# mgaido91/FBK-fairseq-ST

Hardware: AMD Instinct MI355X
Metric: audio-frames/sec (train fwd+bwd) s2t_transformer_m, 80-mel (higher is better)
Workload: dtype bf16

## Files before the change

### fbk_fairseq_st_amd/csrc/attention.hip

```cpp
#include "common.hpp"
#include "prof.hpp"
#include <cstdlib>
#include <type_traits>

template <typename T, int DH> struct ACfg {
    static constexpr int E = Elem<T>::PER16;
    static constexpr int ROWB = DH * (int)sizeof(T);
    static constexpr int NCH = ROWB / 16;
    static constexpr int KG = NCH / 4;
    static constexpr int PROWB = 64 * (int)sizeof(T);
    static constexpr int PCH = PROWB / 16;
    static constexpr int PKG = PCH / 4;
    static constexpr int ND = DH / 16;
    static constexpr int TILE = 64 * ROWB;
    static constexpr int TTILE = DH * PROWB;
    static constexpr int PTILE = 16 * PROWB;
};

__device__ __forceinline__ int swz(int row, int c, int nch) { return c ^ (row & ((nch < 8 ? nch : 8) - 1)); }

template <typename T, int DH>
__device__ __forceinline__ void stage_rows(char* lds, const T* g, long stride, int row0, int nvalid) {
    typedef ACfg<T, DH> C;
    for (int cid = threadIdx.x; cid < 64 * C::NCH; cid += 256) {
// ... 703 lines not shown
        for (int n = 0; n < 4; ++n) { dkT[kb][n] = (f32x4){0.f, 0.f, 0.f, 0.f}; dvT[kb][n] = dkT[kb][n]; }
    const uint32_t drop_th16 = (uint32_t)fminf(p.p_drop * 4294967296.f, 4294967295.f) >> 16;
    const float drop_inv = 1.f / (1.f - p.p_drop);
    const uint32_t drop_ks = drop_seed_key(p.seed), drop_hwm = drop_high_mix(p.seed, 0);
    const uint32_t tkq = (uint32_t)((p.Tk + 3) >> 2);
    const uint32_t drop_thm1x2 = (drop_th16 - 1u) * 0x00010001u;
    const uint32_t own_bit = ((r16 & 1) ? 0x00010000u : 1u) << ((r16 >> 1) & 1);

    const int qstart = p.causal ? bx * 128 : 0;
    const int ntile = qstart < p.Tq ? (p.Tq - qstart + 63) / 64 : 0;
    float* sStat = reinterpret_cast<float*>(smem + 32768);
    auto stage = [&](int qt, int stg) {
        stage2_dma(Qg, p.q_st, dOg, p.do_st, qt, p.Tq, smem + stg * 16384, wave, lane);
        if (wave < 2) {
            float* dst = sStat + stg * 128 + wave * 64;
            if (wave == 1 || qt + lane < p.Tq) {
                const char* sb = reinterpret_cast<const char*>(wave == 0 ? lse : dlt);
                const char* src = sb + (uint32_t)(min(qt + lane, p.Tq - 1) * 4);
                __builtin_amdgcn_global_load_lds((__attribute__((address_space(1))) const void*)src,
                                                 (__attribute__((address_space(3))) void*)dst, 4, 0, 0);
            } else dst[lane] = INFINITY;
        }
    };
    if (ntile > 0) stage(qstart, 0);
    {
        u32x4 kk[4], vv[4];
#pragma unroll
        for (int i = 0; i < 4; ++i) {
            const int cid = threadIdx.x + 256 * i, row = cid >> 3, c = cid & 7;
            const long key = min(bx * 128 + row, p.Tk - 1);
            kk[i] = *reinterpret_cast<const u32x4*>(Kg + key * p.k_st + c * 8);
            vv[i] = *reinterpret_cast<const u32x4*>(Vg + key * p.v_st + c * 8);
        }
#pragma unroll
        for (int i = 0; i < 4; ++i) {
            const int cid = threadIdx.x + 256 * i, row = cid >> 3, c = cid & 7;
            const bool in = bx * 128 + row < klen;
#pragma unroll
            for (int w = 0; w < 4; ++w) { kk[i][w] = in ? kk[i][w] : 0u; vv[i][w] = in ? vv[i][w] : 0u; }
            *reinterpret_cast<u32x4*>(sKown + row * 128 + ((c ^ (row & 7)) << 4)) = kk[i];
            *reinterpret_cast<u32x4*>(sVown + row * 128 + ((c ^ (row & 7)) << 4)) = vv[i];
        }
    }
    S2T_WAIT_VM0();
    __syncthreads();
    const float sc2 = p.scale * 1.44269504088896f;
    const bool generic = p.causal || p.dist_pen;
    ASTAMP(7, 1)
    for (int t = 0; t < ntile; ++t) {
        const int qt = qstart + t * 64;
        const char* sQ = smem + (t & 1) * 16384;
        const char* sDO = sQ + 8192;
        const float* sL = sStat + (t & 1) * 128;
        ASTAMP(t, 0)
        if (t + 1 < ntile) stage(qt + 64, (t + 1) & 1);
        ASTAMP(t, 1)
        auto tile = [&](auto edge_tag, auto drop_tag) {
        constexpr bool EDGE = decltype(edge_tag)::value, DROP = decltype(drop_tag)::value;
#pragma unroll 1
        for (int ib = 0; ib < 2; ++ib) {
        u32x4 pf[2], sf[2];
#pragma unroll
        for (int ii = 0; ii < 2; ++ii) {
            const int i = 2 * ib + ii;
            u32x4 qa[2], da[2];
#pragma unroll
            for (int g = 0; g < 2; ++g) { qa[g] = row_frag128(sQ, 16 * i + r16, 4 * g + q); da[g] = row_frag128(sDO, 16 * i + r16, 4 * g + q); }
            const f32x4 L = *reinterpret_cast<const f32x4*>(sL + 16 * i + 4 * q) * 1.44269504088896f;
            const f32x4 Dl = *reinterpret_cast<const f32x4*>(sL + 64 + 16 * i + 4 * q);
            const uint32_t qrow_quads = DROP ? (uint32_t)(((b * p.H + h) * p.Tq + qt + 16 * i + 4 * q + (r16 & 3))) * tkq : 0u;
#pragma unroll
            for (int kb = 0; kb < 2; ++kb) {
                f32x4 st = {0.f, 0.f, 0.f, 0.f}, dp = {0.f, 0.f, 0.f, 0.f};
#pragma unroll
                for (int g = 0; g < 2; ++g) {
                    const int krow = wave * 32 + 16 * kb + r16;
                    st = mma16<bf16>(qa[g], row_frag128(sKown, krow, 4 * g + q), st);
                    dp = mma16<bf16>(da[g], row_frag128(sVown, krow, 4 * g + q), dp);
                }
                const int key = kw + 16 * kb + r16;
                uint32_t nib = 0u;
                if constexpr (DROP) {
                    const u32x2 hq = drop_hash4_lo(drop_ks, drop_hwm, qrow_quads + ((uint32_t)key >> 2));
                    uint32_t dy, dx, ky, kx;
                    asm("v_pk_sub_u16 %0, %1, %2 clamp" : "=v"(dy) : "v"(hq[1]), "v"(drop_thm1x2));
                    asm("v_pk_sub_u16 %0, %1, %2 clamp" : "=v"(dx) : "v"(hq[0]), "v"(drop_thm1x2));
                    asm("v_pk_min_u16 %0, %1, %2" : "=v"(ky) : "v"(dy), "v"(0x00010001u));
                    asm("v_pk_min_u16 %0, %1, %2" : "=v"(kx) : "v"(dx), "v"(0x00010001u));
                    nib = drop_th16 > 0 ? (ky | (kx << 1)) : 0x00030003u;
                }
                float pv[4], ds[4];
#pragma unroll
                for (int r = 0; r < 4; ++r) {
                    const int qrow = qt + 16 * i + 4 * q + r;
                    float arg = __builtin_fmaf(st[r], sc2, -L[r]);
                    if constexpr (EDGE) { if (p.dist_pen) arg -= dist_pen_log2(qrow, key); }
                    float e = __builtin_amdgcn_exp2f(arg);
                    if constexpr (EDGE) e = (qrow < p.Tq && (!p.causal || key <= qrow)) ? e : 0.f;
                    if constexpr (DROP) {
                        const bool keep = (quad_bcast(nib, r) & own_bit) != 0u;
                        pv[r] = keep ? e : 0.f;
                        ds[r] = e * __builtin_fmaf(keep ? dp[r] : 0.f, drop_inv, -Dl[r]);
                    } else {
                        pv[r] = e;
                        ds[r] = e * (dp[r] - Dl[r]);
                    }
                }
                pf[kb][2 * ii] = pack_bf16(pv[0], pv[1]); pf[kb][2 * ii + 1] = pack_bf16(pv[2], pv[3]);
                sf[kb][2 * ii] = pack_bf16(ds[0], ds[1]); sf[kb][2 * ii + 1] = pack_bf16(ds[2], ds[3]);
            }
        }
#pragma unroll
            for (int n = 0; n < 4; ++n) {
                const u32x4 dot = tr_frag128(sDO, ib, n, r16, q), qtf = tr_frag128(sQ, ib, n, r16, q);
#pragma unroll
                for (int kb = 0; kb < 2; ++kb) {
                    dvT[kb][n] = mma16<bf16>(dot, pf[kb], dvT[kb][n]);
                    dkT[kb][n] = mma16<bf16>(qtf, sf[kb], dkT[kb][n]);
                }
            }
        }
        };
        const bool edge = generic;
        if (p.p_drop > 0.f) { if (edge) tile(std::true_type{}, std::true_type{}); else tile(std::false_type{}, std::true_type{}); }
        else if (edge) tile(std::true_type{}, std::false_type{});
        else tile(std::false_type{}, std::false_type{});
        ASTAMP(t, 3)
        S2T_WAIT_VM0();
        ASTAMP(t, 4)
        __syncthreads();
        ASTAMP(t, 5)
    }
    ASTAMP(7, 2)
    const float dv_scale = p.p_drop > 0.f ? drop_inv : 1.f;
    bf16* dKg = reinterpret_cast<bf16*>(p.dK) + (long)b * p.dk_sb + (long)h * DH;
    bf16* dVg = reinterpret_cast<bf16*>(p.dV) + (long)b * p.dv_sb + (long)h * DH;
#pragma unroll
    for (int kb = 0; kb < 2; ++kb) {
        const int key = kw + 16 * kb + r16;
        if (key >= p.Tk) continue;
        const float kz = key < klen ? 1.f : 0.f;
#pragma unroll
        for (int n = 0; n < 4; ++n) { dkT[kb][n] *= kz * p.scale; dvT[kb][n] *= kz * dv_scale; }
#pragma unroll
        for (int n = 0; n < 4; ++n) {
            u32x2 w;
            w[0] = pack_bf16(dkT[kb][n][0], dkT[kb][n][1]); w[1] = pack_bf16(dkT[kb][n][2], dkT[kb][n][3]);
            *reinterpret_cast<u32x2*>(dKg + (long)key * p.dk_st + 16 * n + 4 * q) = w;
            w[0] = pack_bf16(dvT[kb][n][0], dvT[kb][n][1]); w[1] = pack_bf16(dvT[kb][n][2], dvT[kb][n][3]);
            *reinterpret_cast<u32x2*>(dVg + (long)key * p.dv_st + 16 * n + 4 * q) = w;
        }
    }
    ASTAMP(7, 3)
}

__global__ __launch_bounds__(256, 2) void attn_bwd_dq2_kernel(AttnArgs p) {
    constexpr int DH = 64;
    ASTAMP_EARLY(1)
    extern __shared__ __attribute__((aligned(16))) char smem[];
    const int lane = threadIdx.x & 63, wave = threadIdx.x >> 6, r16 = lane & 15, q = lane >> 4;
    int head;
    const int bx = head_xcd_remap(head, p.B * p.H, gridDim.x);
    const int b = head / p.H, h = head % p.H, qw = bx * 128 + wave * 32;
    const int klen = p.klen ? min(p.klen[b], p.Tk) : p.Tk;
    const bf16* Qg = reinterpret_cast<const bf16*>(p.Q) + (long)b * p.q_sb + (long)h * DH;
    const bf16* Kg = reinterpret_cast<const bf16*>(p.K) + (long)b * p.k_sb + (long)h * DH;
    const bf16* Vg = reinterpret_cast<const bf16*>(p.V) + (long)b * p.v_sb + (long)h * DH;
    const bf16* dOg = reinterpret_cast<const bf16*>(p.dO) + (long)b * p.do_sb + (long)h * DH;
    const float* lse = p.LSE + ((long)b * p.H + h) * p.Tq;
    const float* dlt = p.Delta + ((long)b * p.H + h) * p.Tq;

    int kv_end = klen;
    if (p.causal) kv_end = min(kv_end, bx * 128 + 128);
    const int ntile = (kv_end + 63) / 64;
    if (ntile > 0) stage2_dma(Kg, p.k_st, Vg, p.v_st, 0, p.Tk, smem, wave, lane);
    u32x4 qf[2][2], dof[2][2];
    float L[2], Dl[2];
    const bf16* Og = reinterpret_cast<const bf16*>(p.O) + (long)b * p.o_sb + (long)h * DH;
    u32x4 of[2][2];
#pragma unroll
    for (int qb = 0; qb < 2; ++qb) {
        const long row = min(qw + 16 * qb + r16, p.Tq - 1);
        L[qb] = lse[row] * 1.44269504088896f;
#pragma unroll
        for (int g = 0; g < 2; ++g) {
            qf[qb][g] = *reinterpret_cast<const u32x4*>(Qg + row * p.q_st + (4 * g + q) * 8);
            dof[qb][g] = *reinterpret_cast<const u32x4*>(dOg + row * p.do_st + (4 * g + q) * 8);
            of[qb][g] = *reinterpret_cast<const u32x4*>(Og + row * p.o_st + (4 * g + q) * 8);
        }
    }
#pragma unroll
    for (int qb = 0; qb < 2; ++qb) {
        const int row = qw + 16 * qb + r16;
        const bool in = row < p.Tq;
        float part = 0.f;
#pragma unroll
        for (int g = 0; g < 2; ++g) {
#pragma unroll
            for (int w = 0; w < 4; ++w) { qf[qb][g][w] = in ? qf[qb][g][w] : 0u; dof[qb][g][w] = in ? dof[qb][g][w] : 0u; }
            const bf16* oe = reinterpret_cast<const bf16*>(&of[qb][g]);
            const bf16* de = reinterpret_cast<const bf16*>(&dof[qb][g]);
#pragma unroll
            for (int e = 0; e < 8; ++e) part += (float)oe[e] * (float)de[e];
        }
        L[qb] = in ? L[qb] : 0.f;
        part += __shfl_xor(part, 16); part += __shfl_xor(part, 32);
        Dl[qb] = part;
        if (q == 0 && in) const_cast<float*>(dlt)[row] = part;
    }
    f32x4 dqT[2][4];
#pragma unroll
    for (int qb = 0; qb < 2; ++qb)
#pragma unroll
        for (int n = 0; n < 4; ++n) dqT[qb][n] = (f32x4){0.f, 0.f, 0.f, 0.f};
    const uint32_t drop_th16 = (uint32_t)fminf(p.p_drop * 4294967296.f, 4294967295.f) >> 16;
    const float drop_inv = 1.f / (1.f - p.p_drop);
    const uint32_t drop_ks = drop_seed_key(p.seed), drop_hwm = drop_high_mix(p.seed, 0);
    const uint32_t tkq = (uint32_t)((p.Tk + 3) >> 2);

    const float sc2 = p.scale * 1.44269504088896f;
    const bool generic = p.causal || p.dist_pen;
    S2T_WAIT_VM0();
    __syncthreads();
    ASTAMP(7, 1)
    for (int t = 0; t < ntile; ++t) {
        const int kv0 = t * 64;
        const char* sK = smem + (t & 1) * 16384;
        const char* sV = sK + 8192;
        ASTAMP(t, 0)
        if (t + 1 < ntile) stage2_dma(Kg, p.k_st, Vg, p.v_st, kv0 + 64, p.Tk, smem + ((t + 1) & 1) * 16384, wave, lane);
        ASTAMP(t, 1)
        u32x4 sf[2][2];
        auto ds_tile = [&](auto edge_tag, auto drop_tag, auto tail_tag) {
        constexpr bool EDGE = decltype(edge_tag)::value, DROP = decltype(drop_tag)::value, TAIL = decltype(tail_tag)::value;
        const int tail_thr = klen - kv0 - 4 * q;
#pragma unroll
        for (int j = 0; j < 4; ++j) {
            u32x4 ka[2], va[2];
#pragma unroll
            for (int g = 0; g < 2; ++g) { ka[g] = row_frag128(sK, 16 * j + r16, 4 * g + q); va[g] = row_frag128(sV, 16 * j + r16, 4 * g + q); }
#pragma unroll
            for (int qb = 0; qb < 2; ++qb) {
                f32x4 st = {0.f, 0.f, 0.f, 0.f}, dp = {0.f, 0.f, 0.f, 0.f};
#pragma unroll
                for (int g = 0; g < 2; ++g) { st = mma16<bf16>(ka[g], qf[qb][g], st); dp = mma16<bf16>(va[g], dof[qb][g], dp); }
                const int qrow = qw + 16 * qb + r16;
                const int key0 = kv0 + 16 * j + 4 * q;
                u32x2 hq = {0u, 0u};
                if constexpr (DROP) hq = drop_hash4_lo(drop_ks, drop_hwm, (uint32_t)((b * p.H + h) * p.Tq + qrow) * tkq + ((uint32_t)key0 >> 2));
                float ds[4];
#pragma unroll
                for (int r = 0; r < 4; ++r) {
                    float arg = __builtin_fmaf(st[r], sc2, -L[qb]);
                    if constexpr (EDGE) { if (p.dist_pen) arg -= dist_pen_log2(qrow, key0 + r); }
                    float e = __builtin_amdgcn_exp2f(arg);
                    if constexpr (EDGE) {
                        const int key = key0 + r;
                        e = (key < klen && (!p.causal || key <= qrow)) ? e : 0.f;
                    }
                    if constexpr (TAIL) e = (16 * j + r < tail_thr) ? e : 0.f;
                    if constexpr (DROP) ds[r] = e * __builtin_fmaf(drop_field(hq, r) >= drop_th16 ? dp[r] : 0.f, drop_inv, -Dl[qb]);
                    else ds[r] = e * (dp[r] - Dl[qb]);
                }
                sf[qb][j >> 1][2 * (j & 1)] = pack_bf16(ds[0], ds[1]); sf[qb][j >> 1][2 * (j & 1) + 1] = pack_bf16(ds[2], ds[3]);
            }
        }
        };
        const bool tail = kv0 + 64 > klen;
        if (generic) { if (p.p_drop > 0.f) ds_tile(std::true_type{}, std::true_type{}, std::false_type{}); else ds_tile(std::true_type{}, std::false_type{}, std::false_type{}); }
        else if (p.p_drop > 0.f) { if (tail) ds_tile(std::false_type{}, std::true_type{}, std::true_type{}); else ds_tile(std::false_type{}, std::true_type{}, std::false_type{}); }
        else if (tail) ds_tile(std::false_type{}, std::false_type{}, std::true_type{});
        else ds_tile(std::false_type{}, std::false_type{}, std::false_type{});
        ASTAMP(t, 2)
#pragma unroll
        for (int jb = 0; jb < 2; ++jb)
#pragma unroll
            for (int n = 0; n < 4; ++n) {
                const u32x4 kt = tr_frag128(sK, jb, n, r16, q);
#pragma unroll
                for (int qb = 0; qb < 2; ++qb) dqT[qb][n] = mma16<bf16>(kt, sf[qb][jb], dqT[qb][n]);
            }
        ASTAMP(t, 3)
        S2T_WAIT_VM0();
        ASTAMP(t, 4)
        __syncthreads();
        ASTAMP(t, 5)
    }
    ASTAMP(7, 2)
    bf16* dQg = reinterpret_cast<bf16*>(p.dQ) + (long)b * p.dq_sb + (long)h * DH;
#pragma unroll
    for (int qb = 0; qb < 2; ++qb) {
        const int qrow = qw + 16 * qb + r16;
        if (qrow >= p.Tq) continue;
#pragma unroll
        for (int n = 0; n < 4; ++n) {
            u32x2 w;
            w[0] = pack_bf16(dqT[qb][n][0] * p.scale, dqT[qb][n][1] * p.scale); w[1] = pack_bf16(dqT[qb][n][2] * p.scale, dqT[qb][n][3] * p.scale);
            *reinterpret_cast<u32x2*>(dQg + (long)qrow * p.dq_st + 16 * n + 4 * q) = w;
        }
    }
    ASTAMP(7, 3)
}

static bool span32(long stride, int rows) {
    return stride >= 0 && stride * 2 < (1l << 24) && (long)rows * stride * 2 + 256 < (1l << 32);
}
static bool strides_ok(int dtype, const long* s, int n) {
    const int e = dtype == S2T_BF16 ? 8 : 4;
    for (int i = 0; i < n; ++i) if (s[i] % e) return false;
    return true;
}

template <typename T, int DH> static int fwd_launch(const AttnArgs& a, hipStream_t st) {
    typedef ACfg<T, DH> C;
    dim3 grid((a.Tq + 63) / 64, a.H, a.B);
    const size_t lds = 2 * C::TILE + 4 * C::PTILE;
    hipLaunchKernelGGL((attn_fwd_kernel<T, DH>), grid, dim3(256), lds, st, a);
    S2T_LAUNCH_CHECK();
    return S2T_OK;
}
template <typename T, int DH> static int bwd_launch(const AttnArgs& a, hipStream_t st) {
    typedef ACfg<T, DH> C;
    const long rows = (long)a.B * a.H * a.Tq;
    bool dkv2 = false, dq2 = false;
    if constexpr (sizeof(T) == 2 && DH == 64) {
        const bool v1 = g_s2t_opt_attn_v1 != 0;
        const bool al = !(a.dk_st % 4) && !(a.dk_sb % 4) && !(a.dv_st % 4) && !(a.dv_sb % 4) && !(a.dq_st % 4) && !(a.dq_sb % 4) &&
                        !((uintptr_t)a.dK & 7) && !((uintptr_t)a.dV & 7) && !((uintptr_t)a.dQ & 7);
        const bool idx32 = (unsigned long long)a.B * a.H * a.Tq * (unsigned long long)((a.Tk + 3) & ~3) < (1ull << 34);
        dkv2 = !v1 && al && idx32 && a.Tk >= 128 && span32(a.q_st, a.Tq) && span32(a.do_st, a.Tq);
        dq2 = !v1 && al && idx32 && span32(a.k_st, a.Tk) && span32(a.v_st, a.Tk) && (a.Tq >= 128 || (a.Tq >= S2T_ATTN_V2_MIN_TQ && a.Tk >= 128)) && !(a.o_st % 8) && !(a.o_sb % 8) && !((uintptr_t)a.O & 15);
        if (dq2) {
            hipLaunchKernelGGL(attn_bwd_dq2_kernel, dim3((a.Tq + 127) / 128, a.H, a.B), dim3(256), 32768, st, a);
            S2T_LAUNCH_CHECK();
        } else {
            hipLaunchKernelGGL((attn_delta_kernel<T, DH>), dim3((unsigned)((rows * 16 + 255) / 256)), dim3(256), 0, st, a);
            S2T_LAUNCH_CHECK();
        }
        if (dkv2) {
            {
                static bool attr = false;
                if (!attr) { (void)hipFuncSetAttribute(reinterpret_cast<const void*>(&attn_bwd_dkv2_kernel), hipFuncAttributeMaxDynamicSharedMemorySize, 32768 + 1024 + 32768); attr = true; }
            }
            hipLaunchKernelGGL(attn_bwd_dkv2_kernel, dim3((a.Tk + 127) / 128, a.H, a.B), dim3(256), 32768 + 1024 + 32768, st, a);
            S2T_LAUNCH_CHECK();
        }
    } else {
        hipLaunchKernelGGL((attn_delta_kernel<T, DH>), dim3((unsigned)((rows * 16 + 255) / 256)), dim3(256), 0, st, a);
        S2T_LAUNCH_CHECK();
    }
    if (!dkv2) {
        static bool attr = false;
        const size_t lds = 4 * C::TILE + 8 * C::PTILE;
        if (!attr && lds > 65536) {
            (void)hipFuncSetAttribute(reinterpret_cast<const void*>(&attn_bwd_dkv_kernel<T, DH>), hipFuncAttributeMaxDynamicSharedMemorySize, (int)lds);
            attr = true;
        }
        hipLaunchKernelGGL((attn_bwd_dkv_kernel<T, DH>), dim3((a.Tk + 63) / 64, a.H, a.B), dim3(256), lds, st, a);
        S2T_LAUNCH_CHECK();
    }
    if (!dq2) {
        static bool attr = false;
        const size_t lds = 3 * C::TILE + 4 * C::PTILE;
        if (!attr && lds > 65536) {
            (void)hipFuncSetAttribute(reinterpret_cast<const void*>(&attn_bwd_dq_kernel<T, DH>), hipFuncAttributeMaxDynamicSharedMemorySize, (int)lds);
            attr = true;
        }
        hipLaunchKernelGGL((attn_bwd_dq_kernel<T, DH>), dim3((a.Tq + 63) / 64, a.H, a.B), dim3(256), lds, st, a);
        S2T_LAUNCH_CHECK();
    }
    return S2T_OK;
}

static int check_common(int dtype, int head_dim, const AttnArgs& a) {
    if (dtype != S2T_F32 && dtype != S2T_BF16) return S2T_ENOTSUP;
    if (head_dim != 64 && head_dim != 32) return S2T_ENOTSUP;
    if (a.B <= 0 || a.H <= 0 || a.Tq <= 0 || a.Tk <= 0) return S2T_EINVAL;
    if (a.p_drop < 0.f || a.p_drop >= 1.f || (a.dist_pen != 0 && a.dist_pen != 1)) return S2T_EINVAL;
    return S2T_OK;
}

extern "C" int s2t_attn_fwd(int dtype, int head_dim, int B, int H, int Tq, int Tk,
                            const void* Q, long q_st, long q_sb, const void* K, long k_st, long k_sb,
                            const void* V, long v_st, long v_sb, void* O, long o_st, long o_sb, float* LSE,
                            const int* klen, int causal, int dist_penalty, float scale, float p_drop, unsigned long long seed,
                            void* stream) {
    AttnArgs a{};
    a.dist_pen = dist_penalty;
    a.Q = Q; a.K = K; a.V = V; a.O = O; a.LSE = LSE;
    a.q_st = q_st; a.q_sb = q_sb; a.k_st = k_st; a.k_sb = k_sb; a.v_st = v_st; a.v_sb = v_sb; a.o_st = o_st; a.o_sb = o_sb;
    a.klen = klen; a.B = B; a.H = H; a.Tq = Tq; a.Tk = Tk; a.causal = causal; a.scale = scale; a.p_drop = p_drop; a.seed = seed;
    if (B == 0 || Tq == 0) return S2T_OK;
    int rc = check_common(dtype, head_dim, a);
    if (rc) return rc;
    if (!Q || !K || !V || !O) return S2T_EINVAL;
    const long s[] = {q_st, q_sb, k_st, k_sb, v_st, v_sb};
    if (!strides_ok(dtype, s, 6)) return S2T_EINVAL;
    hipStream_t st = (hipStream_t)stream;
    ProfScope prof("attn_fwd", st, 4.0 * B * H * (double)Tq * Tk * head_dim * (causal ? 0.5 : 1.0), 0.0);
    if (dtype == S2T_BF16 && head_dim == 64 && (Tq >= 128 || (Tq >= S2T_ATTN_V2_MIN_TQ && Tk >= 128)) && (o_st % 4) == 0 && (o_sb % 4) == 0 && ((uintptr_t)O & 7) == 0) {
        const bool v1 = g_s2t_opt_attn_v1 != 0 || !span32(k_st, Tk) || !span32(v_st, Tk);
        if (!v1) {
            hipLaunchKernelGGL(attn_fwd2_kernel, dim3((Tq + 127) / 128, H, B), dim3(256), 32768 + 512 + 16384, st, a);
            S2T_LAUNCH_CHECK();
            return S2T_OK;
        }
    }
    if (dtype == S2T_BF16) return head_dim == 64 ? fwd_launch<bf16, 64>(a, st) : fwd_launch<bf16, 32>(a, st);
    return head_dim == 64 ? fwd_launch<float, 64>(a, st) : fwd_launch<float, 32>(a, st);
}

extern "C" int s2t_attn_bwd(int dtype, int head_dim, int B, int H, int Tq, int Tk,
                            const void* Q, long q_st, long q_sb, const void* K, long k_st, long k_sb,
                            const void* V, long v_st, long v_sb, const void* O, long o_st, long o_sb,
                            const void* dO, long do_st, long do_sb, const float* LSE, float* Delta,
                            void* dQ, long dq_st, long dq_sb, void* dK, long dk_st, long dk_sb,
                            void* dV, long dv_st, long dv_sb,
                            const int* klen, int causal, int dist_penalty, float scale, float p_drop, unsigned long long seed,
                            void* stream) {
    AttnArgs a{};
    a.dist_pen = dist_penalty;
    a.Q = Q; a.K = K; a.V = V; a.O = const_cast<void*>(O); a.LSE = const_cast<float*>(LSE);
    a.dO = dO; a.dQ = dQ; a.dK = dK; a.dV = dV; a.Delta = Delta;
    a.q_st = q_st; a.q_sb = q_sb; a.k_st = k_st; a.k_sb = k_sb; a.v_st = v_st; a.v_sb = v_sb; a.o_st = o_st; a.o_sb = o_sb;
    a.dq_st = dq_st; a.dq_sb = dq_sb; a.dk_st = dk_st; a.dk_sb = dk_sb; a.dv_st = dv_st; a.dv_sb = dv_sb; a.do_st = do_st; a.do_sb = do_sb;
    a.klen = klen; a.B = B; a.H = H; a.Tq = Tq; a.Tk = Tk; a.causal = causal; a.scale = scale; a.p_drop = p_drop; a.seed = seed;
    if (B == 0 || Tq == 0) return S2T_OK;
    int rc = check_common(dtype, head_dim, a);
    if (rc) return rc;
    if (!Q || !K || !V || !O || !dO || !LSE || !Delta || !dQ || !dK || !dV) return S2T_EINVAL;
    const long s[] = {q_st, q_sb, k_st, k_sb, v_st, v_sb, do_st, do_sb};
    if (!strides_ok(dtype, s, 8)) return S2T_EINVAL;
    hipStream_t st = (hipStream_t)stream;
    ProfScope prof("attn_bwd", st, 14.0 * B * H * (double)Tq * Tk * head_dim * (causal ? 0.5 : 1.0), 0.0);
    if (dtype == S2T_BF16) return head_dim == 64 ? bwd_launch<bf16, 64>(a, st) : bwd_launch<bf16, 32>(a, st);
    return head_dim == 64 ? bwd_launch<float, 64>(a, st) : bwd_launch<float, 32>(a, st);
}

template <typename T>
__global__ __launch_bounds__(256) void attn_probs_avg_kernel(const T* __restrict__ Q, long q_st, long q_sb, const T* __restrict__ Kp, long k_st,
                                                             long k_sb, const int* __restrict__ klen, float* __restrict__ out, int H, int dh,
                                                             int Tq, int Tk, int heads_used, float scale) {
    __shared__ float sh[16];
    __shared__ float qs[128];
    const int tq = blockIdx.x, b = blockIdx.y;
    const int kl = klen ? min(klen[b], Tk) : Tk;
    constexpr int NK = 8;
    float acc[NK];
#pragma unroll
    for (int i = 0; i < NK; ++i) acc[i] = 0.f;
    for (int h = 0; h < heads_used; ++h) {
        __syncthreads();
        if ((int)threadIdx.x < dh) qs[threadIdx.x] = to_f32(Q[tq * q_st + b * q_sb + h * dh + threadIdx.x]) * scale;
        __syncthreads();
        float s[NK];
        float m = -INFINITY;
#pragma unroll
        for (int i = 0; i < NK; ++i) {
            const int tk = threadIdx.x + 256 * i;
            s[i] = -INFINITY;
            if (tk < kl) {
                const T* kr = Kp + (long)tk * k_st + b * k_sb + h * dh;
                float d = 0.f;
                for (int j = 0; j < dh; ++j) d += qs[j] * to_f32(kr[j]);
                s[i] = d;
            }
            m = fmaxf(m, s[i]);
        }
        m = block_max(m, sh);
        float l = 0.f;
#pragma unroll
        for (int i = 0; i < NK; ++i) { s[i] = (s[i] == -INFINITY) ? 0.f : expf(s[i] - m); l += s[i]; }
        l = block_sum(l, sh);
        const float inv = l > 0.f ? 1.f / (l * heads_used) : 0.f;
#pragma unroll
        for (int i = 0; i < NK; ++i) acc[i] += s[i] * inv;
    }
#pragma unroll
    for (int i = 0; i < NK; ++i) {
        const int tk = threadIdx.x + 256 * i;
        if (tk < Tk) out[((long)b * Tq + tq) * Tk + tk] = acc[i];
    }
}

extern "C" int s2t_attn_probs_avg(int dtype, int head_dim, int B, int H, int Tq, int Tk, const void* Q, long q_st, long q_sb,
                                  const void* K, long k_st, long k_sb, const int* klen, int heads_used, float scale, float* out,
                                  void* stream) {
    if (B == 0 || Tq == 0 || Tk == 0) return S2T_OK;
    if (!Q || !K || !out || head_dim <= 0 || head_dim > 128 || H <= 0 || heads_used <= 0 || heads_used > H) return S2T_EINVAL;
    if (Tk > 2048) return S2T_ENOTSUP;
    hipStream_t st = (hipStream_t)stream;
    dim3 grid((unsigned)Tq, (unsigned)B);
    if (dtype == S2T_BF16) hipLaunchKernelGGL(attn_probs_avg_kernel<bf16>, grid, dim3(256), 0, st, (const bf16*)Q, q_st, q_sb, (const bf16*)K, k_st, k_sb,
                                               klen, out, H, head_dim, Tq, Tk, heads_used, scale);
    else if (dtype == S2T_F32) hipLaunchKernelGGL(attn_probs_avg_kernel<float>, grid, dim3(256), 0, st, (const float*)Q, q_st, q_sb, (const float*)K, k_st,
                                                  k_sb, klen, out, H, head_dim, Tq, Tk, heads_used, scale);
    else return S2T_ENOTSUP;
    S2T_LAUNCH_CHECK();
    return S2T_OK;
}
```

Measured before the change: 6.853 million.

## Add single-block-per-head attention kernels for short query sequences

Adds specialized forward and backward attention kernels for Tq<=64 (e.g., decoder self-attention) in which one 256-thread block handles a whole (batch, head). The backward kernel fuses the delta computation, dK/dV and dQ into one launch, keeping dQ in registers and reducing it across waves through LDS, so no separate delta kernel or second pass over K/V is needed. This targets launch overhead and redundant passes for small decoder shapes. The trade-off is fewer blocks (B*H) and so less parallelism on large GPUs, with all of Tk handled serially inside each block.

```diff
diff --git a/fbk_fairseq_st_amd/csrc/attention.hip b/fbk_fairseq_st_amd/csrc/attention.hip
--- a/fbk_fairseq_st_amd/csrc/attention.hip
+++ b/fbk_fairseq_st_amd/csrc/attention.hip
@@ -1029,6 +1029,371 @@
     ASTAMP(7, 3)
 }
 
+__global__ __launch_bounds__(256, 2) void attn_fwd_sq_kernel(AttnArgs p) {
+    constexpr int DH = 64;
+    extern __shared__ __attribute__((aligned(16))) char smem[];
+    const int lane = threadIdx.x & 63, wave = __builtin_amdgcn_readfirstlane(threadIdx.x >> 6), r16 = lane & 15, q = lane >> 4;
+    const int head = blockIdx.x, b = head / p.H, h = head % p.H, qw = wave * 16;
+    const bool active = qw < p.Tq;
+    const int klen = p.klen ? min(p.klen[b], p.Tk) : p.Tk;
+    const bf16* Qg = reinterpret_cast<const bf16*>(p.Q) + (long)b * p.q_sb + (long)h * DH;
+    const bf16* Kg = reinterpret_cast<const bf16*>(p.K) + (long)b * p.k_sb + (long)h * DH;
+    const bf16* Vg = reinterpret_cast<const bf16*>(p.V) + (long)b * p.v_sb + (long)h * DH;
+
+    f32x4 o[4];
+#pragma unroll
+    for (int n = 0; n < 4; ++n) o[n] = (f32x4){0.f, 0.f, 0.f, 0.f};
+    float m = -INFINITY, l = 0.f;
+    int kv_end = klen;
+    if (p.causal) kv_end = min(kv_end, p.Tq);
+    const int ntile = kv_end > 0 ? (kv_end + 63) / 64 : 0;
+
+    const uint32_t kst2 = (uint32_t)p.k_st * 2u, vst2 = (uint32_t)p.v_st * 2u;
+    auto stage = [&](int kv0, char* st) {
+#pragma unroll
+        for (int i = 0; i < 2; ++i) {
+            const int r8 = 8 * (wave + 4 * i), row = r8 + (lane >> 3), pos = lane & 7;
+            const uint32_t r = (uint32_t)min(kv0 + row, p.Tk - 1);
+            char* dst = st + r8 * 128;
+            const char* ka = reinterpret_cast<const char*>(Kg) + (__umul24(r, kst2) + (uint32_t)((pos ^ (row & 7)) << 4));
+            const char* va = reinterpret_cast<const char*>(Vg) + (__umul24(r, vst2) + (uint32_t)((pos ^ (row & 6)) << 4));
+            __builtin_amdgcn_global_load_lds((__attribute__((address_space(1))) const void*)ka, (__attribute__((address_space(3))) void*)dst, 16, 0, 0);
+            __builtin_amdgcn_global_load_lds((__attribute__((address_space(1))) const void*)va, (__attribute__((address_space(3))) void*)(dst + 8192), 16, 0, 0);
+        }
+    };
+    const uint32_t drop_th16 = (uint32_t)fminf(p.p_drop * 4294967296.f, 4294967295.f) >> 16;
+    const uint32_t drop_thm1x2 = (drop_th16 - 1u) * 0x00010001u;
+    const bool has_drop = drop_th16 > 0;
+    const float drop_inv = 1.f / (1.f - p.p_drop);
+    const uint32_t drop_ks = drop_seed_key(p.seed), drop_hwm = drop_high_mix(p.seed, 0);
+    const uint32_t tkq = (uint32_t)((p.Tk + 3) >> 2);
+    const float sc2 = p.scale * 1.44269504088896f;
+
+    float* sInit = reinterpret_cast<float*>(smem + 32768);
+    if (threadIdx.x < 128) {
+        const int i = threadIdx.x & 63;
+        sInit[threadIdx.x] = (threadIdx.x < 64 || (ntile - 1) * 64 + i < klen) ? 0.f : -INFINITY;
+    }
+    if (ntile > 0) stage(0, smem);
+    char* sQ = smem + 32768 + 512;
+#pragma unroll
+    for (int i = 0; i < 2; ++i) {
+        const int r8 = 8 * (wave + 4 * i), row = r8 + (lane >> 3), pos = lane & 7;
+        const long r = min(row, p.Tq - 1);
+        __builtin_amdgcn_global_load_lds((__attribute__((address_space(1))) const void*)(Qg + r * p.q_st + ((pos ^ (row & 7)) << 3)),
+                                         (__attribute__((address_space(3))) void*)(sQ + r8 * 128), 16, 0, 0);
+    }
+    S2T_WAIT_VM0();
+    __syncthreads();
+    const int qrow = qw + r16;
+    const uint32_t qrow_quads = (uint32_t)((b * p.H + h) * p.Tq + qrow) * tkq;
+    for (int t = 0; t < ntile; ++t) {
+        const int kv0 = t * 64;
+        const char* sK = smem + (t & 1) * 16384;
+        const char* sV = sK + 8192;
+        if (t + 1 < ntile) stage(kv0 + 64, smem + ((t + 1) & 1) * 16384);
+        if (active) {
+            f32x4 s[4];
+            const float* sInit0 = sInit + ((!p.causal && t == ntile - 1) ? 64 : 0) + 4 * q;
+            u32x4 qf[2];
+#pragma unroll
+            for (int g = 0; g < 2; ++g) qf[g] = row_frag128(sQ, qw + r16, 4 * g + q);
+#pragma unroll
+            for (int j = 0; j < 4; ++j) {
+                s[j] = *reinterpret_cast<const f32x4*>(sInit0 + 16 * j);
+#pragma unroll
+                for (int g = 0; g < 2; ++g) s[j] = mma16<bf16>(row_frag128(sK, 16 * j + r16, 4 * g + q), qf[g], s[j]);
+            }
+            u32x4 pf[2];
+            auto softmax_tile = [&](auto mask_tag, auto drop_tag) {
+                constexpr bool MASK = decltype(mask_tag)::value, DROP = decltype(drop_tag)::value;
+                float mx = -INFINITY;
+#pragma unroll
+                for (int j = 0; j < 4; ++j) {
+                    if constexpr (MASK) {
+#pragma unroll
+                        for (int r = 0; r < 4; ++r) {
+                            const int key = kv0 + 16 * j + 4 * q + r;
+                            s[j][r] = (key < klen && key <= qrow) ? s[j][r] : -INFINITY;
+                        }
+                    }
+                    mx = fmaxf(fmaxf(mx, s[j][0]), s[j][1]);
+                    mx = fmaxf(fmaxf(mx, s[j][2]), s[j][3]);
+                }
+                mx = max_over_rows(mx);
+                const float mn = fmaxf(m, mx * sc2);
+                const float mu = (mn == -INFINITY) ? 0.f : mn;
+                const float alpha = __builtin_amdgcn_exp2f(m - mu);
+                m = mn;
+                f32x2_t rs2 = {0.f, 0.f};
+                const uint32_t qlo = qrow_quads + (uint32_t)((kv0 + 4 * q) >> 2);
+#pragma unroll
+                for (int j = 0; j < 4; ++j) {
+                    float pv[4];
+#pragma unroll
+                    for (int r = 0; r < 4; ++r) pv[r] = __builtin_amdgcn_exp2f(__builtin_fmaf(s[j][r], sc2, -mu));
+                    rs2 += (f32x2_t){pv[0], pv[1]};
+                    rs2 += (f32x2_t){pv[2], pv[3]};
+                    uint32_t p01 = pack_bf16(pv[0], pv[1]), p23 = pack_bf16(pv[2], pv[3]);
+                    if constexpr (DROP) {
+                        const u32x2 hq = drop_hash4_lo(drop_ks, drop_hwm, qlo + 4u * j);
+                        p01 = drop_pair(p01, hq[1], drop_thm1x2); p23 = drop_pair(p23, hq[0], drop_thm1x2);
+                    }
+                    pf[j >> 1][2 * (j & 1)] = p01;
+                    pf[j >> 1][2 * (j & 1) + 1] = p23;
+                }
+                l = l * alpha + (rs2[0] + rs2[1]);
+#pragma unroll
+                for (int n = 0; n < 4; ++n) o[n] *= alpha;
+            };
+            if (p.causal) { if (has_drop) softmax_tile(std::true_type{}, std::true_type{}); else softmax_tile(std::true_type{}, std::false_type{}); }
+            else if (has_drop) softmax_tile(std::false_type{}, std::true_type{});
+            else softmax_tile(std::false_type{}, std::false_type{});
+#pragma unroll
+            for (int kb = 0; kb < 2; ++kb)
+#pragma unroll
+                for (int n = 0; n < 4; ++n) {
+                    u32x4 vf;
+#pragma unroll
+                    for (int hh = 0; hh < 2; ++hh) {
+                        const int row = 32 * kb + 16 * hh + 4 * q + (r16 >> 2);
+                        const int ch = 2 * n + ((r16 & 3) >> 1);
+                        const char* a = sV + row * 128 + ((ch ^ (row & 6)) << 4) + ((r16 & 1) << 3);
+                        const s16x4_t v = __builtin_amdgcn_ds_read_tr16_b64_v4i16((__attribute__((address_space(3))) s16x4_t*)a);
+                        const u32x2 w = __builtin_bit_cast(u32x2, v);
+                        vf[2 * hh] = w[0]; vf[2 * hh + 1] = w[1];
+                    }
+                    o[n] = mma16<bf16>(vf, pf[kb], o[n]);
+                }
+        }
+        S2T_WAIT_VM0();
+        __syncthreads();
+    }
+    float lt = l;
+    lt += __shfl_xor(lt, 16); lt += __shfl_xor(lt, 32);
+    if (qrow >= p.Tq) return;
+    bf16* Og = reinterpret_cast<bf16*>(p.O) + (long)b * p.o_sb + (long)h * DH;
+    const float inv = lt > 0.f ? drop_inv / lt : 0.f;
+#pragma unroll
+    for (int n = 0; n < 4; ++n) {
+        u32x2 w;
+        w[0] = pack_bf16(o[n][0] * inv, o[n][1] * inv);
+        w[1] = pack_bf16(o[n][2] * inv, o[n][3] * inv);
+        *reinterpret_cast<u32x2*>(Og + (long)qrow * p.o_st + 16 * n + 4 * q) = w;
+    }
+    if (q == 0 && p.LSE) p.LSE[((long)b * p.H + h) * p.Tq + qrow] = m * 0.693147180559945f + logf(lt);
+}
+
+#define S2T_SQ_TPITCH 136
+#define S2T_SQ_BWD_LDS (16384 + 512 + 32768 + 4 * 16 * S2T_SQ_TPITCH)
+__global__ __launch_bounds__(256, 2) void attn_bwd_sq_kernel(AttnArgs p) {
+    constexpr int DH = 64;
+    extern __shared__ __attribute__((aligned(16))) char smem[];
+    const int lane = threadIdx.x & 63, wave = __builtin_amdgcn_readfirstlane(threadIdx.x >> 6), r16 = lane & 15, q = lane >> 4;
+    const int head = blockIdx.x, b = head / p.H, h = head % p.H;
+    const int klen = p.klen ? min(p.klen[b], p.Tk) : p.Tk;
+    const bf16* Qg = reinterpret_cast<const bf16*>(p.Q) + (long)b * p.q_sb + (long)h * DH;
+    const bf16* Kg = reinterpret_cast<const bf16*>(p.K) + (long)b * p.k_sb + (long)h * DH;
+    const bf16* Vg = reinterpret_cast<const bf16*>(p.V) + (long)b * p.v_sb + (long)h * DH;
+    const bf16* dOg = reinterpret_cast<const bf16*>(p.dO) + (long)b * p.do_sb + (long)h * DH;
+    const bf16* Og = reinterpret_cast<const bf16*>(p.O) + (long)b * p.o_sb + (long)h * DH;
+    bf16* dKg = reinterpret_cast<bf16*>(p.dK) + (long)b * p.dk_sb + (long)h * DH;
+    bf16* dVg = reinterpret_cast<bf16*>(p.dV) + (long)b * p.dv_sb + (long)h * DH;
+    const float* lse = p.LSE + ((long)b * p.H + h) * p.Tq;
+    float* dlt = const_cast<float*>(p.Delta) + ((long)b * p.H + h) * p.Tq;
+    const char* sQ = smem;
+    const char* sDO = smem + 8192;
+    float* sStat = reinterpret_cast<float*>(smem + 16384);
+    char* sKV = smem + 16384 + 512;
+    char* sT = sKV + 32768 + wave * (16 * S2T_SQ_TPITCH);
+
+    int kv_end = klen;
+    if (p.causal) kv_end = min(kv_end, p.Tq);
+    const int ntile = kv_end > 0 ? (kv_end + 63) / 64 : 0;
+    const int nq = (p.Tq + 15) >> 4;
+    if (ntile > 0) stage2_dma(Kg, p.k_st, Vg, p.v_st, 0, p.Tk, sKV, wave, lane);
+    stage2_dma(Qg, p.q_st, dOg, p.do_st, 0, p.Tq, smem, wave, lane);
+    {
+        const int row = threadIdx.x >> 2, seg = threadIdx.x & 3;
+        const long rc = min(row, p.Tq - 1);
+        u32x4 of[2], df[2];
+#pragma unroll
+        for (int g = 0; g < 2; ++g) {
+            of[g] = *reinterpret_cast<const u32x4*>(Og + rc * p.o_st + 16 * seg + 8 * g);
+            df[g] = *reinterpret_cast<const u32x4*>(dOg + rc * p.do_st + 16 * seg + 8 * g);
+        }
+        const float L = lse[rc];
+        float part = 0.f;
+#pragma unroll
+        for (int g = 0; g < 2; ++g) {
+            const bf16* oe = reinterpret_cast<const bf16*>(&of[g]);
+            const bf16* de = reinterpret_cast<const bf16*>(&df[g]);
+#pragma unroll
+            for (int e = 0; e < 8; ++e) part += (float)oe[e] * (float)de[e];
+        }
+        part += __shfl_xor(part, 1); part += __shfl_xor(part, 2);
+        if (seg == 0) {
+            const bool in = row < p.Tq;
+            sStat[row] = in ? L * 1.44269504088896f : INFINITY;
+            sStat[64 + row] = in ? part : 0.f;
+            if (in) dlt[row] = part;
+        }
+    }
+    f32x4 dq[4][4];
+#pragma unroll
+    for (int i = 0; i < 4; ++i)
+#pragma unroll
+        for (int n = 0; n < 4; ++n) dq[i][n] = (f32x4){0.f, 0.f, 0.f, 0.f};
+    const uint32_t drop_th16 = (uint32_t)fminf(p.p_drop * 4294967296.f, 4294967295.f) >> 16;
+    const float drop_inv = 1.f / (1.f - p.p_drop);
+    const uint32_t drop_ks = drop_seed_key(p.seed), drop_hwm = drop_high_mix(p.seed, 0);
+    const uint32_t tkq = (uint32_t)((p.Tk + 3) >> 2);
+    const uint32_t drop_thm1x2 = (drop_th16 - 1u) * 0x00010001u;
+    const uint32_t own_bit = ((r16 & 1) ? 0x00010000u : 1u) << ((r16 >> 1) & 1);
+    const float sc2 = p.scale * 1.44269504088896f;
+    const float dv_scale = p.p_drop > 0.f ? drop_inv : 1.f;
+    S2T_WAIT_VM0();
+    __syncthreads();
+    for (int t = 0; t < ntile; ++t) {
+        const int kv0 = t * 64;
+        const char* sK = sKV + (t & 1) * 16384;
+        const char* sV = sK + 8192;
+        if (t + 1 < ntile) stage2_dma(Kg, p.k_st, Vg, p.v_st, kv0 + 64, p.Tk, sKV + ((t + 1) & 1) * 16384, wave, lane);
+        const int key = kv0 + 16 * wave + r16;
+        f32x4 dkT[4], dvT[4];
+#pragma unroll
+        for (int n = 0; n < 4; ++n) { dkT[n] = (f32x4){0.f, 0.f, 0.f, 0.f}; dvT[n] = dkT[n]; }
+        auto tile = [&](auto mask_tag, auto drop_tag) {
+            constexpr bool MASK = decltype(mask_tag)::value, DROP = decltype(drop_tag)::value;
+            u32x4 kfr[2], vfr[2];
+#pragma unroll
+            for (int g = 0; g < 2; ++g) { kfr[g] = row_frag128(sK, 16 * wave + r16, 4 * g + q); vfr[g] = row_frag128(sV, 16 * wave + r16, 4 * g + q); }
+#pragma unroll
+            for (int ib = 0; ib < 2; ++ib) {
+                if (2 * ib >= nq) break;
+                u32x4 pf = {0u, 0u, 0u, 0u}, sf = {0u, 0u, 0u, 0u};
+#pragma unroll
+                for (int ii = 0; ii < 2; ++ii) {
+                    const int i = 2 * ib + ii;
+                    if (i >= nq) break;
+                    u32x4 qa[2], da[2];
+#pragma unroll
+                    for (int g = 0; g < 2; ++g) { qa[g] = row_frag128(sQ, 16 * i + r16, 4 * g + q); da[g] = row_frag128(sDO, 16 * i + r16, 4 * g + q); }
+                    const f32x4 L = *reinterpret_cast<const f32x4*>(sStat + 16 * i + 4 * q);
+                    const f32x4 Dl = *reinterpret_cast<const f32x4*>(sStat + 64 + 16 * i + 4 * q);
+                    f32x4 st = {0.f, 0.f, 0.f, 0.f}, dp = {0.f, 0.f, 0.f, 0.f};
+#pragma unroll
+                    for (int g = 0; g < 2; ++g) { st = mma16<bf16>(qa[g], kfr[g], st); dp = mma16<bf16>(da[g], vfr[g], dp); }
+                    uint32_t nib = 0u;
+                    if constexpr (DROP) {
+                        const uint32_t qrow_quads = (uint32_t)((b * p.H + h) * p.Tq + 16 * i + 4 * q + (r16 & 3)) * tkq;
+                        const u32x2 hq = drop_hash4_lo(drop_ks, drop_hwm, qrow_quads + ((uint32_t)key >> 2));
+                        uint32_t dy, dx, ky, kx;
+                        asm("v_pk_sub_u16 %0, %1, %2 clamp" : "=v"(dy) : "v"(hq[1]), "v"(drop_thm1x2));
+                        asm("v_pk_sub_u16 %0, %1, %2 clamp" : "=v"(dx) : "v"(hq[0]), "v"(drop_thm1x2));
+                        asm("v_pk_min_u16 %0, %1, %2" : "=v"(ky) : "v"(dy), "v"(0x00010001u));
+                        asm("v_pk_min_u16 %0, %1, %2" : "=v"(kx) : "v"(dx), "v"(0x00010001u));
+                        nib = drop_th16 > 0 ? (ky | (kx << 1)) : 0x00030003u;
+                    }
+                    float pv[4], ds[4];
+#pragma unroll
+                    for (int r = 0; r < 4; ++r) {
+                        float e = __builtin_amdgcn_exp2f(__builtin_fmaf(st[r], sc2, -L[r]));
+                        if constexpr (MASK) e = (key < klen && (!p.causal || key <= 16 * i + 4 * q + r)) ? e : 0.f;
+                        if constexpr (DROP) {
+                            const bool keep = (quad_bcast(nib, r) & own_bit) != 0u;
+                            pv[r] = keep ? e : 0.f;
+                            ds[r] = e * __builtin_fmaf(keep ? dp[r] : 0.f, drop_inv, -Dl[r]);
+                        } else {
+                            pv[r] = e;
+                            ds[r] = e * (dp[r] - Dl[r]);
+                        }
+                    }
+                    pf[2 * ii] = pack_bf16(pv[0], pv[1]); pf[2 * ii + 1] = pack_bf16(pv[2], pv[3]);
+                    sf[2 * ii] = pack_bf16(ds[0], ds[1]); sf[2 * ii + 1] = pack_bf16(ds[2], ds[3]);
+                    *reinterpret_cast<u32x2*>(sT + r16 * S2T_SQ_TPITCH + (16 * i + 4 * q) * 2) = (u32x2){sf[2 * ii], sf[2 * ii + 1]};
+                }
+#pragma unroll
+                for (int n = 0; n < 4; ++n) {
+                    const u32x4 dot = tr_frag128(sDO, ib, n, r16, q), qtf = tr_frag128(sQ, ib, n, r16, q);
+                    dvT[n] = mma16<bf16>(dot, pf, dvT[n]);
+                    dkT[n] = mma16<bf16>(qtf, sf, dkT[n]);
+                }
+            }
+            asm volatile("s_waitcnt lgkmcnt(0)" ::: "memory");
+            __builtin_amdgcn_wave_barrier();
+            s16x4_t kt[4];
+#pragma unroll
+            for (int n = 0; n < 4; ++n) {
+                const int row = 16 * wave + 4 * q + (r16 >> 2), ch = 2 * n + ((r16 & 3) >> 1);
+                kt[n] = __builtin_amdgcn_ds_read_tr16_b64_v4i16((__attribute__((address_space(3))) s16x4_t*)(sK + row * 128 + ((ch ^ (row & 7)) << 4) + ((r16 & 1) << 3)));
+            }
+#pragma unroll
+            for (int i = 0; i < 4; ++i) {
+                if (i >= nq) break;
+                const s16x4_t a = __builtin_amdgcn_ds_read_tr16_b64_v4i16(
+                    (__attribute__((address_space(3))) s16x4_t*)(sT + (4 * q + (r16 >> 2)) * S2T_SQ_TPITCH + (16 * i + 4 * (r16 & 3)) * 2));
+#pragma unroll
+                for (int n = 0; n < 4; ++n) dq[i][n] = __builtin_amdgcn_mfma_f32_16x16x16bf16_1k(a, kt[n], dq[i][n], 0, 0, 0);
+            }
+            asm volatile("" ::: "memory");
+        };
+        if (kv0 + 16 * wave < kv_end) {
+            const bool mask = p.causal || kv0 + 64 > klen;
+            if (p.p_drop > 0.f) { if (mask) tile(std::true_type{}, std::true_type{}); else tile(std::false_type{}, std::true_type{}); }
+            else if (mask) tile(std::true_type{}, std::false_type{});
+            else tile(std::false_type{}, std::false_type{});
+        }
+        S2T_WAIT_VM0();
+        __syncthreads();
+        if (key < p.Tk) {
+#pragma unroll
+            for (int n = 0; n < 4; ++n) {
+                dkT[n] *= p.scale; dvT[n] *= dv_scale;
+                u32x2 w;
+                w[0] = pack_bf16(dkT[n][0], dkT[n][1]); w[1] = pack_bf16(dkT[n][2], dkT[n][3]);
+                *reinterpret_cast<u32x2*>(dKg + (long)key * p.dk_st + 16 * n + 4 * q) = w;
+                w[0] = pack_bf16(dvT[n][0], dvT[n][1]); w[1] = pack_bf16(dvT[n][2], dvT[n][3]);
+                *reinterpret_cast<u32x2*>(dVg + (long)key * p.dv_st + 16 * n + 4 * q) = w;
+            }
+        }
+    }
+    for (int key = ntile * 64 + (threadIdx.x >> 3); key < p.Tk; key += 32) {
+        const int c = (threadIdx.x & 7) * 8;
+        *reinterpret_cast<u32x2*>(dKg + (long)key * p.dk_st + c) = (u32x2){0u, 0u};
+        *reinterpret_cast<u32x2*>(dKg + (long)key * p.dk_st + c + 4) = (u32x2){0u, 0u};
+        *reinterpret_cast<u32x2*>(dVg + (long)key * p.dv_st + c) = (u32x2){0u, 0u};
+        *reinterpret_cast<u32x2*>(dVg + (long)key * p.dv_st + c + 4) = (u32x2){0u, 0u};
+    }
+    float* red = reinterpret_cast<float*>(sKV);
+    bf16* dQg = reinterpret_cast<bf16*>(p.dQ) + (long)b * p.dq_sb + (long)h * DH;
+#pragma unroll
+    for (int half = 0; half < 2; ++half) {
+        if (half) __syncthreads();
+#pragma unroll
+        for (int i = 0; i < 4; ++i) {
+            if (i >= nq) break;
+#pragma unroll
+            for (int nn = 0; nn < 2; ++nn)
+#pragma unroll
+                for (int r = 0; r < 4; ++r) red[(wave * 64 + 16 * i + 4 * q + r) * 32 + 16 * nn + r16] = dq[i][2 * half + nn][r];
+        }
+        __syncthreads();
+        const int row = threadIdx.x >> 2, c = (threadIdx.x & 3) * 8;
+        if (row < p.Tq) {
+            f32x4 s0 = {0.f, 0.f, 0.f, 0.f}, s1 = s0;
+#pragma unroll
+            for (int w = 0; w < 4; ++w) {
+                s0 += *reinterpret_cast<const f32x4*>(red + (w * 64 + row) * 32 + c);
+                s1 += *reinterpret_cast<const f32x4*>(red + (w * 64 + row) * 32 + c + 4);
+            }
+            s0 *= p.scale; s1 *= p.scale;
+            *reinterpret_cast<u32x2*>(dQg + (long)row * p.dq_st + 32 * half + c) = (u32x2){pack_bf16(s0[0], s0[1]), pack_bf16(s0[2], s0[3])};
+            *reinterpret_cast<u32x2*>(dQg + (long)row * p.dq_st + 32 * half + c + 4) = (u32x2){pack_bf16(s1[0], s1[1]), pack_bf16(s1[2], s1[3])};
+        }
+    }
+}
+
 static bool span32(long stride, int rows) {
     return stride >= 0 && stride * 2 < (1l << 24) && (long)rows * stride * 2 + 256 < (1l << 32);
 }
@@ -1036,6 +1401,21 @@
     const int e = dtype == S2T_BF16 ? 8 : 4;
     for (int i = 0; i < n; ++i) if (s[i] % e) return false;
     return true;
+}
+
+static bool sq_shape(const AttnArgs& a) {
+    if (g_s2t_opt_attn_v1 != 0 || a.dist_pen || a.Tq > 64) return false;
+    if (!((a.Tq >= S2T_ATTN_V2_MIN_TQ && a.Tk >= 128) || (a.causal && a.Tq == a.Tk))) return false;
+    const bool idx32 = (unsigned long long)a.B * a.H * a.Tq * (unsigned long long)((a.Tk + 3) & ~3) < (1ull << 34);
+    return idx32 && span32(a.k_st, a.Tk) && span32(a.v_st, a.Tk);
+}
+static bool sq_fwd_route(const AttnArgs& a) {
+    return sq_shape(a) && !(a.o_st % 4) && !(a.o_sb % 4) && !((uintptr_t)a.O & 7);
+}
+static bool sq_bwd_route(const AttnArgs& a) {
+    const bool al = !(a.dk_st % 4) && !(a.dk_sb % 4) && !(a.dv_st % 4) && !(a.dv_sb % 4) && !(a.dq_st % 4) && !(a.dq_sb % 4) &&
+                    !((uintptr_t)a.dK & 7) && !((uintptr_t)a.dV & 7) && !((uintptr_t)a.dQ & 7);
+    return sq_shape(a) && al && span32(a.q_st, a.Tq) && span32(a.do_st, a.Tq) && !(a.o_st % 8) && !(a.o_sb % 8) && !((uintptr_t)a.O & 15);
 }
 
 template <typename T, int DH> static int fwd_launch(const AttnArgs& a, hipStream_t st) {
@@ -1051,6 +1431,11 @@
     const long rows = (long)a.B * a.H * a.Tq;
     bool dkv2 = false, dq2 = false;
     if constexpr (sizeof(T) == 2 && DH == 64) {
+        if (sq_bwd_route(a)) {
+            hipLaunchKernelGGL(attn_bwd_sq_kernel, dim3((unsigned)(a.B * a.H)), dim3(256), S2T_SQ_BWD_LDS, st, a);
+            S2T_LAUNCH_CHECK();
+            return S2T_OK;
+        }
         const bool v1 = g_s2t_opt_attn_v1 != 0;
         const bool al = !(a.dk_st % 4) && !(a.dk_sb % 4) && !(a.dv_st % 4) && !(a.dv_sb % 4) && !(a.dq_st % 4) && !(a.dq_sb % 4) &&
                         !((uintptr_t)a.dK & 7) && !((uintptr_t)a.dV & 7) && !((uintptr_t)a.dQ & 7);
@@ -1125,6 +1510,11 @@
     if (!strides_ok(dtype, s, 6)) return S2T_EINVAL;
     hipStream_t st = (hipStream_t)stream;
     ProfScope prof("attn_fwd", st, 4.0 * B * H * (double)Tq * Tk * head_dim * (causal ? 0.5 : 1.0), 0.0);
+    if (dtype == S2T_BF16 && head_dim == 64 && sq_fwd_route(a)) {
+        hipLaunchKernelGGL(attn_fwd_sq_kernel, dim3((unsigned)(B * H)), dim3(256), 32768 + 512 + 8192, st, a);
+        S2T_LAUNCH_CHECK();
+        return S2T_OK;
+    }
     if (dtype == S2T_BF16 && head_dim == 64 && (Tq >= 128 || (Tq >= S2T_ATTN_V2_MIN_TQ && Tk >= 128)) && (o_st % 4) == 0 && (o_sb % 4) == 0 && ((uintptr_t)O & 7) == 0) {
         const bool v1 = g_s2t_opt_attn_v1 != 0 || !span32(k_st, Tk) || !span32(v_st, Tk);
         if (!v1) {
@@ -1159,7 +1549,8 @@
     const long s[] = {q_st, q_sb, k_st, k_sb, v_st, v_sb, do_st, do_sb};
     if (!strides_ok(dtype, s, 8)) return S2T_EINVAL;
     hipStream_t st = (hipStream_t)stream;
-    ProfScope prof("attn_bwd", st, 14.0 * B * H * (double)Tq * Tk * head_dim * (causal ? 0.5 : 1.0), 0.0);
+    const bool sq = dtype == S2T_BF16 && head_dim == 64 && sq_bwd_route(a);
+    ProfScope prof("attn_bwd", st, (sq ? 10.0 : 14.0) * B * H * (double)Tq * Tk * head_dim * (causal ? 0.5 : 1.0), 0.0);
     if (dtype == S2T_BF16) return head_dim == 64 ? bwd_launch<bf16, 64>(a, st) : bwd_launch<bf16, 32>(a, st);
     return head_dim == 64 ? bwd_launch<float, 64>(a, st) : bwd_launch<float, 32>(a, st);
 }
```

Result: faster. 6.955 million, median of 6 (+1.5%).
